# SZU-AdvTech-2022/165-Learning-based-Multi-modality-Image-and-Video-Compression

Hardware: AMD Instinct MI355X
Metric: 256×256 patches/sec (RD-loss fwd+bwd) at 1/2/4/8 GPUs; PSNR/bpp parity (higher is better)
Workload: dtype bf16; 1 GPU; bmshj2018-hyperprior q1 B=16 256x256 RD-loss training step (fwd+bwd+clip+Adam+aux), HIP-graph replay; model=bmshj2018-hyperprior, quality=1, global_batch=16, per_gpu_batch=16, patch=256, parallelism=dp1

## Files before the change

### 165-learning-based-multi-modality-image-and-video-compression_amd/compressai/_native.py

```python
from __future__ import annotations

import ctypes
import os
from ctypes import POINTER, Structure, c_char_p, c_float, c_int, c_int32, c_int64, c_size_t, c_void_p

_PKG_ROOT = os.path.dirname(os.path.dirname(os.path.abspath(__file__)))
LIB_PATH = os.environ.get("CAI_LIB", os.path.join(_PKG_ROOT, "lib", "libcai.so"))

CAI_OK, CAI_EINVAL, CAI_EDEVICE, CAI_EWORKSPACE = 0, 1, 2, 3
F32, BF16 = 0, 1
ACT_NONE, ACT_RELU, ACT_LEAKY = 0, 1, 2
MASK_NONE, MASK_POS, MASK_LEAKY, MASK_SIGN = 0, 1, 2, 3
MASK_BEFORE_RES = 16
Q_NOISE, Q_DEQUANTIZE, Q_SYMBOLS = 0, 1, 2
ADAM_CLIP, ADAM_SKIP_NONFINITE, ADAM_ZERO_GRAD = 1, 2, 4
ADAM_SMALL_N = 1 << 16


class ConvGeom(Structure):
    _fields_ = [(n, c_int32) for n in (
        "batch", "in_c", "in_h", "in_w", "out_c", "out_h", "out_w",
        "kernel", "stride", "pad", "output_padding", "transposed")]


# ... 62 lines not shown
                ("out", c_void_p), ("gc", c_void_p), ("gb", c_void_p), ("ga", c_void_p), ("res2", c_void_p),
                ("xmask", c_void_p), ("x_ld", c_int32), ("y_ld", c_int32), ("out_ld", c_int32),
                ("res2_ld", c_int32), ("xmask_ld", c_int32), ("kpa", c_int32), ("kpb", c_int32), ("kpc", c_int32),
                ("gy_masked", c_int32)]


class ResunitWgradArgs(Structure):
    _fields_ = [("batch", c_int32), ("h", c_int32), ("w", c_int32), ("n", c_int32),
                ("x", c_void_p), ("h1", c_void_p), ("h2", c_void_p), ("ga", c_void_p), ("gb", c_void_p),
                ("gc", c_void_p), ("x_ld", c_int32), ("gc_ld", c_int32), ("dwa", c_void_p), ("dba", c_void_p),
                ("dwb", c_void_p), ("dbb", c_void_p), ("dwc", c_void_p), ("dbc", c_void_p), ("accumulate", c_int32)]


_P, _I, _I64, _F, _S = c_void_p, c_int, c_int64, c_float, c_size_t
_G = POINTER(ConvGeom)
_N = POINTER(NoiseSrc)
SIGNATURES = {
    "cai_last_error": (c_char_p, []),
    "cai_version": (c_int, []),
    "cai_abi_count": (c_int, []),
    "cai_conv_packed_weight_bytes": (_S, [_G, _I, _I]),
    "cai_conv_pack_weight": (_I, [_G, _I, _I, _P, _P, _P, _P]),
    "cai_conv_pack_desc_bytes": (_S, []),
    "cai_conv_pack_describe": (_I, [_G, _I, _I, _P, _P, _P, _P]),
    "cai_conv_pack_finalize": (_I64, [_P, c_int32]),
    "cai_conv_pack_many": (_I, [_P, c_int32, _I, _I64, _P]),
    "cai_pack_nchw": (_I, [_P, c_int32, c_int32, c_int32, c_int32, _I, _P, c_int32, _P]),
    "cai_conv_workspace_bytes": (_S, [_G, _I, _I]),
    "cai_conv_fwd": (_I, [_G, _I, _P, c_int32, c_int32, _P, _P, c_int32, _F, _P, _I, _I64, _I64, _I64, _I64,
                          _P, _S, _P]),
    "cai_conv_fwd_res": (_I, [_G, _I, _P, c_int32, c_int32, _P, _P, c_int32, _F, _P, c_int32, _P, _I, _I64, _I64,
                              _I64, _I64, _P, _S, _P]),
    "cai_conv_gdn_fwd": (_I, [_G, _I, _P, c_int32, c_int32, _P, _P, _P, _I64, _I64, _I64, _I64, _P, _P, c_int32, _P,
                              c_int32, _P, _S, _P]),
    "cai_conv_gdn_fused": (c_int32, [_G, _I, c_int32]),
    "cai_conv_gdn_kernel_name": (c_char_p, [_G, _I, c_int32, c_int32]),
    "cai_conv_dgrad": (_I, [_G, _I, _P, c_int32, _P, _P, c_int32, c_int32, _F, _P, c_int32, _P, _S, _P]),
    "cai_conv_dgrad_res": (_I, [_G, _I, _P, c_int32, _P, _P, c_int32, _P, c_int32, c_int32, _F, _P, c_int32, _P, _S,
                                _P]),
    "cai_conv_dgrad_res2": (_I, [_G, _I, _P, c_int32, _P, _P, c_int32, _P, c_int32, _P, c_int32, c_int32, _F, _P,
                                 c_int32, _P, _S, _P]),
    "cai_conv_wgrad_workspace_bytes": (_S, [_G, _I]),
    "cai_resunit": (_I, [POINTER(ResunitArgs), c_int32, _P]),
    "cai_resunit_wgrad_workspace_bytes": (_S, [POINTER(ResunitWgradArgs)]),
    "cai_resunit_wgrad": (_I, [POINTER(ResunitWgradArgs), _P, _S, _P, POINTER(ReduceJob)]),
    "cai_conv_kernel_name": (c_char_p, [_G, _I, _I, c_int32]),
    "cai_conv_split_factor": (c_int32, [_G, _I, _I, c_int32]),
    "cai_conv_wgrad": (_I, [_G, _I, _P, c_int32, c_int32, c_int32, _P, c_int32, _P, _P, c_int32, _P, _S, _P]),
    "cai_conv_wgrad_deferred": (_I, [_G, _I, _P, c_int32, c_int32, c_int32, _P, c_int32, _P, _P, c_int32, _P, _S, _P,
                                     POINTER(ReduceJob)]),
    "cai_reduce_jobs": (_I, [POINTER(ReduceJob), c_int32, _P]),
    "cai_reduce_jobs_grid": (_I, [POINTER(ReduceJob), c_int32, c_int32, _P]),
    "cai_conv_wgrad_batch": (_I, [POINTER(WgradCall), c_int32, _P, POINTER(ReduceJob)]),
    "cai_resunit_wgrad_batch": (_I, [POINTER(ResunitWgradArgs), POINTER(c_void_p), POINTER(c_size_t), c_int32, _P,
                                    POINTER(ReduceJob)]),
    "cai_deconv_small_workspace_bytes": (_S, [_G, _I]),
    "cai_deconv_small_fwd": (_I, [_G, _I, _P, c_int32, _P, _P, _P, _P, _S, _P]),
    "cai_deconv_small_bwd": (_I, [_G, _I, _P, c_int32, _P, _P, _P, c_int32, _P, _P, c_int32, _P, _S, _P]),
    "cai_edge_supported": (_I, [_G, _I]),
    "cai_edge_workspace_bytes": (_S, [_G, _I]),
    "cai_edge_frag_bytes": (_S, [_G, _I, _I]),
    "cai_edge_pack_weights": (_I, [_G, _I, _I, _P, _P, _P]),
    "cai_edge_pack_describe": (_I, [_G, _I, _I, _P, _P, _P]),
    "cai_edge_conv_fwd": (_I, [_G, _P, _P, _P, _P, c_int32, _P]),
    "cai_edge_conv_gdn_fwd": (_I, [_G, _P, _P, _P, _P, c_int32, _P, _P, _P, c_int32, _P]),
    "cai_edge_conv_gdn_fused": (c_int32, [_G]),
    "cai_edge_deconv_fwd": (_I, [_G, _P, c_int32, _P, _P, _P, _P]),
    "cai_edge_deconv_dgrad": (_I, [_G, _P, _P, _P, c_int32, _P]),
    "cai_edge_wgrad": (_I, [_G, _P, _P, c_int32, _P, _P, c_int32, _P, _S, _P]),
    "cai_edge_wgrad_deferred": (_I, [_G, _P, _P, c_int32, _P, _P, c_int32, _P, _S, _P, POINTER(ReduceJob)]),
    "cai_add_act": (_I, [_I, _P, c_int32, _P, c_int32, _P, c_int32, _I64, c_int32, c_int32, _F, _P]),
    "cai_axpy_dev": (_I, [_I64, _P, _P, _P, _P]),
    "cai_act": (_I, [_I, _P, c_int32, _P, c_int32, _I64, c_int32, c_int32, _F, _P]),
    "cai_gdn1_out": (_I, [_I, _P, c_int32, _P, c_int32, _P, c_int32, _I64, c_int32, c_int32, _P]),
    "cai_gdn1_out_bwd": (_I, [_I, _P, c_int32, _P, c_int32, _P, c_int32, _P, c_int32, _P, c_int32, _I64, c_int32,
                              c_int32, _P]),
    "cai_gate_fwd": (_I, [_I, _P, _P, _P, _P, c_int32, _I64, c_int32, _P]),
    "cai_gate_bwd": (_I, [_I, _P, _P, _P, c_int32, _P, _P, c_int32, _I64, c_int32, c_int32, _P]),
    "cai_pixel_shuffle": (_I, [_I, _P, POINTER(c_int64), _P, POINTER(c_int64), c_int32, c_int32, c_int32, c_int32,
                               c_int32, c_int32, _P]),
    "cai_layernorm_fwd": (_I, [_I, _P, c_int32, _I64, c_int32, _P, _P, _F, _P, c_int32, _P, _P, _P]),
    "cai_layernorm_bwd_workspace_bytes": (_S, [_I64, c_int32]),
    "cai_layernorm_bwd": (_I, [_I, _P, c_int32, _P, c_int32, _I64, c_int32, _P, _P, _P, _P, c_int32, _P, _P, c_int32,
                               _P, _S, _P]),
    "cai_gelu_fwd": (_I, [_I, _P, c_int32, _P, c_int32, _I64, c_int32, _P]),
    "cai_gelu_bwd": (_I, [_I, _P, c_int32, _P, c_int32, _P, c_int32, _I64, c_int32, _P]),
    "cai_window_attn_fwd": (_I, [_I, POINTER(WindowAttn), _P, c_int32, _P]),
    "cai_window_attn_bwd_workspace_bytes": (_S, [POINTER(WindowAttn)]),
    "cai_window_attn_bwd": (_I, [_I, POINTER(WindowAttn), _P, c_int32, _P, c_int32, _P, c_int32, _P, c_int32, _P, _S,
                                 _P]),
    "cai_channel_mean_workspace_bytes": (_S, [c_int32, _I64, c_int32]),
    "cai_channel_mean": (_I, [_I, _P, c_int32, _P, c_int32, c_int32, _I64, c_int32, _P, _F, _P, _S, _P]),
    "cai_channel_affine": (_I, [_I, _P, c_int32, _P, _P, _F, _P, c_int32, c_int32, _I64, c_int32, _P]),
    "cai_gdn_reparam": (_I, [_P, _P, c_int32, _F, _F, _I, _P, _P, _P]),
    "cai_gdn_reparam_describe": (_I, [_P, _P, c_int32, _F, _F, _P, _P, _P]),
    "cai_gdn_fwd": (_I, [_I, _P, c_int32, _I64, c_int32, _P, _P, c_int32, _P, c_int32, _P]),
    "cai_gdn_bwd": (_I, [_I, _P, c_int32, _P, c_int32, _I64, c_int32, _P, _P, c_int32, _P, c_int32, _P, _P]),
    "cai_gdn_param_grad_workspace_bytes": (_S, [_I64, c_int32, _I]),
    "cai_gdn_param_grad": (_I, [_I, _P, c_int32, _P, _I64, c_int32, _P, _P, _F, _F, _P, _P, c_int32, _P, _S, _P]),
    "cai_gdn_backward_workspace_bytes": (_S, [_I64, c_int32, _I]),
    "cai_gdn_kernel_name": (c_char_p, [_I, _I64, c_int32, c_int32, c_int32, c_int32]),
    "cai_gdn_backward": (_I, [_I, _P, c_int32, _P, c_int32, _I64, c_int32, _P, _P, c_int32, _P, c_int32, _P, _P, _F, _F,
                              _P, _P, c_int32, _P, _S, _P]),
    "cai_gdn_backward_deferred": (_I, [_I, _P, c_int32, _P, c_int32, _I64, c_int32, _P, _P, c_int32, _P, c_int32, _P,
                                       _P, _F, _F, _P, _P, c_int32, _P, _S, _P, POINTER(ReduceJob)]),
    "cai_uniform_noise": (_I, [_P, _I64, _P, _P]),
# ... 83 lines not shown
```

### 165-learning-based-multi-modality-image-and-video-compression_amd/compressai/_ops.py

```python
from __future__ import annotations

import ctypes
import math
import os
import warnings
from typing import Optional, Sequence, Tuple

import torch

from . import _ledger
from ._native import (ACT_LEAKY, ACT_NONE, ACT_RELU, BF16, F32, MASK_BEFORE_RES, MASK_LEAKY, MASK_NONE, MASK_POS,
                      Q_DEQUANTIZE, Q_NOISE,
                      GC_SCALES_RELU, JOB_EDGE, JOB_GDN, JOB_NONE, JOB_WGRAD, NOISE_BUF, NOISE_DRAW, NOISE_REPLAY, ArArgs, ConvGeom, EbGrads, EbParams, NoiseSrc, RdGrads,
                      RdInputs, ReduceJob, ResunitArgs, ResunitWgradArgs, WgradCall, lib)

_VP = ctypes.c_void_p
_GDN_TWO_PASS = os.environ.get("CAI_GDN_TWO_PASS", "0") == "1"
_RD_UNFUSED = os.environ.get("CAI_RD_UNFUSED", "0") == "1"
_EDGE_OFF = os.environ.get("CAI_EDGE_OFF", "0") == "1"



DIRECT_GRAD_ATTR = "_cai_direct_grad"

# ... 703 lines not shown
            fan, done = getattr(ctx, "fan", None), False
            if fan is not None and fan.pending is not None and dres is None and dt == torch.bfloat16 and ldx % 8 == 0:
                post = fan.pending
                if aux is None:
                    dres, fan.pending = post, None
                elif "halo" not in _conv_kernel(g, dt, 1)():
                    ppm, pld = to_pm(post, dt, 4)
                    mode = spec.in_mask | MASK_BEFORE_RES
                    _ledger.run(lambda ppm=ppm, dx=dx, wt=wt, gpm=gpm, ws=ws: lib.cai_conv_dgrad_res(
                                    ctypes.byref(g), code, _p(gpm), gld, _p(wt), _p(ppm), pld, _p(dx), ldx, mode,
                                    spec.in_mask_param, _p(xpm), ctx.xld, _p(ws), wsb, st),
                                "conv_dgrad", _conv_kernel(g, dt, 1), fl, nb + post.numel() * _es(dt), dt,
                                _ledger.shape_of(g))
                    fan.pending, done = None, True
            if done:
                pass
            elif dres is not None and dt == torch.bfloat16 and aux is None and ldx % 8 == 0:
                rpm, rld = to_pm(dres, dt, 4)
                maux = xpm if rmask != MASK_NONE else None
                if dres2 is not None:
                    r2pm, r2ld = to_pm(dres2, dt, 4)
                    _ledger.run(lambda: lib.cai_conv_dgrad_res2(ctypes.byref(g), code, _p(gpm), gld, _p(wt), _p(rpm),
                                                                rld, _p(r2pm), r2ld, _p(dx), ldx, rmask, 0.0,
                                                                _p(maux), ctx.xld if maux is not None else 0, _p(ws),
                                                                wsb, st),
                                "conv_dgrad", _conv_kernel(g, dt, 1), fl, nb, dt, _ledger.shape_of(g))
                else:
                    _ledger.run(lambda: lib.cai_conv_dgrad_res(ctypes.byref(g), code, _p(gpm), gld, _p(wt), _p(rpm),
                                                               rld, _p(dx), ldx, rmask, 0.0, _p(maux),
                                                               ctx.xld if maux is not None else 0, _p(ws), wsb, st),
                                "conv_dgrad", _conv_kernel(g, dt, 1), fl, nb, dt, _ledger.shape_of(g))
            else:
                _ledger.run(lambda: lib.cai_conv_dgrad(ctypes.byref(g), code, _p(gpm), gld, _p(wt), _p(dx), ldx,
                                                       spec.in_mask, spec.in_mask_param, _p(aux),
                                                       ctx.xld if aux is not None else 0, _p(ws), wsb, st),
                            "conv_dgrad", _conv_kernel(g, dt, 1), fl, nb, dt, _ledger.shape_of(g))
                if dres is not None:
                    dx = dx + dres
                if dres2 is not None:
                    dx = dx + dres2
                if rmask != MASK_NONE:
                    raise RuntimeError("conv dgrad: a residual-gradient mask needs the fused bf16 path")
        if ctx.needs_input_grad[1] or (ctx.has_bias and ctx.needs_input_grad[2]):
            wparam, bparam = ctx.params
            dw, db = conv_wgrad(g, dt, xpm, ctx.xld, int(spec.in_abs), gpm, gld, wparam, bparam, weight,
                                ctx.has_bias)
        dres = None
        if ctx.has_res and ctx.needs_input_grad[4]:
            dres = gpm
        return dx, dw, db, None, dres


_BATCHED_WGRAD = {}
_BATCHED_WGRAD_KERNELS = (b"wgrad_small_kernel", b"wgrad_glds_kernel<256>", b"wgrad_glds_kernel<128>",
                          b"wgrad_halo_kernel<3,s1>")


def _small_wgrad(g, code, in_abs) -> bool:
    key = (tuple(getattr(g, f) for f, _ in ConvGeom._fields_), code, int(in_abs))
    v = _BATCHED_WGRAD.get(key)
    if v is None:
        name = lib.cai_conv_kernel_name(ctypes.byref(g), code, 2, int(in_abs))
        v = _BATCHED_WGRAD[key] = name in _BATCHED_WGRAD_KERNELS
    return v


def conv_wgrad(g, dt, xpm, xld, in_abs, gpm, gld, wparam, bparam, weight, has_bias):
    code = dcode(dt)
    dev = gpm.device
    nbytes = lib.cai_conv_wgrad_workspace_bytes(ctypes.byref(g), code)
    wbase = getattr(wparam, "_base", None)
    wdir = wparam if direct_grad(wparam) else (
        wbase if wbase is not None and wbase.numel() == wparam.numel() and direct_grad(wbase) else None)
    direct = wdir is not None and (bparam is None or direct_grad(bparam))
    if direct:
        dw = wdir.grad if wdir is wparam else wdir.grad.view(wparam.shape)
        db = bparam.grad if bparam is not None else None
    else:
        dw = torch.empty(weight.shape, dtype=torch.float32, device=dev)
        db = torch.empty(g.out_c, dtype=torch.float32, device=dev) if has_bias else None
    fl, nb = _ledger.conv_cost(g, _es(dt), 2)
    st = _stream()
    if defer_reduce_ok(direct) and _WGRAD_BATCH and not _WGRAD_SIDE_PX and _small_wgrad(g, code, in_abs):
        wws = torch.empty(nbytes, dtype=torch.uint8, device=dev)
        call = WgradCall(g, code, _p(xpm), xld, int(in_abs), 0, _p(gpm), gld, _p(dw), _p(db), 1, _p(wws), nbytes)
        defer_wgrad_call(call, dev, xpm, gpm, wws)
    elif defer_reduce_ok(direct):
        npix = g.batch * (g.in_h * g.in_w if g.transposed else g.out_h * g.out_w)
        with _SideDeferred(dev, npix, xpm, gpm):
            wws = torch.empty(nbytes, dtype=torch.uint8, device=dev)
            job = ReduceJob()
            lib.cai_conv_wgrad_deferred(ctypes.byref(g), code, _p(xpm), xld, int(in_abs), 0, _p(gpm), gld, _p(dw),
                                        _p(db), 1, _p(wws), nbytes, _stream(), ctypes.byref(job))
            defer_job(job, dev, wws)
    else:
        with _WgradLaunch(dev, direct, xpm, gpm):
            wws = torch.empty(nbytes, dtype=torch.uint8, device=dev)
            sw = _stream()
            _ledger.run(lambda: lib.cai_conv_wgrad(ctypes.byref(g), code, _p(xpm), xld, int(in_abs), 0, _p(gpm), gld,
                                                   _p(dw), _p(db), int(direct), _p(wws), nbytes, sw),
                        "conv_wgrad", _conv_kernel(g, dt, 2, in_abs), fl, nb, dt, _ledger.shape_of(g))
    if direct:
        return None, None
    if weight.dtype != torch.float32:
        dw = dw.to(weight.dtype)
    return dw, db


# ... 1491 lines not shown
```

### 165-learning-based-multi-modality-image-and-video-compression_amd/csrc/conv.hip

```cpp
#include "common.hpp"

#include <type_traits>
#include "edge_frag.hpp"
#include "gdn_tile.hpp"
#include "mfma.hpp"
#include "reduce_jobs.hpp"
#include "conv_args.hpp"

#include <algorithm>
#include <vector>

namespace cai {

constexpr int NT = 256;


__device__ __forceinline__ int swz(int row, int slot) { return slot ^ ((row >> 1) & 7); }

__device__ __forceinline__ float apply_act(float v, int act, float prm) {
    if (act == CAI_ACT_RELU) return v > 0.f ? v : 0.f;
    if (act == CAI_ACT_LEAKY) return v > 0.f ? v : v * prm;
    return v;
}
__device__ __forceinline__ float act_pre(const ConvArgs& a, float v) {
// ... 3116 lines not shown
        one(std::integral_constant<int, 1>());
        one(std::integral_constant<int, 2>());
        one(std::integral_constant<int, 3>());
    }
    if constexpr ((FLAGS & WG_BIAS) != 0) {
        if (do_bias) {
#pragma unroll
            for (int tm = 0; tm < TMR; ++tm) {
                if ((tm & 3) != wc) continue;
                float v = bsum[tm];
                v += __shfl_xor(v, 16);
                v += __shfl_xor(v, 32);
                const int n = r0 + wr * (16 * TMR) + tm * 16 + lane;
                if (lane < 16 && n < a.Ng) a.bws[(int64_t)split * a.Ng + n] = v;
            }
        }
    }
    if constexpr ((FLAGS & WG_TBIAS) != 0) {
#pragma unroll
        for (int t = 0; t < W::TN; ++t) {
            float v = tsum[t];
            v += __shfl_xor(v, 16);
            v += __shfl_xor(v, 32);
            const int col = wcol + t * 16 + (lane & 15);
            if (lane < 16 && tsel[t] >= 0)
                a.bws[((int64_t)split * a.tb_s * a.tb_s + tsel[t]) * a.nbias + q0 + col % 64] = v;
        }
    }
#pragma unroll
    for (int tn = 0; tn < W::TN; ++tn) {
        const int col = wcol + tn * 16 + (lane & 15), kw = col / 64;
        const int gcol = (kh * KS + kw) * a.Cq_pad + q0 + col % 64;
#pragma unroll
        for (int tm = 0; tm < TMR; ++tm)
#pragma unroll
            for (int r = 0; r < 4; ++r) {
                const int row = r0 + wr * (16 * TMR) + tm * 16 + (lane >> 4) * 4 + r;
                if (row < a.Ng) out[(int64_t)row * a.ncols + gcol] = acc[tm][tn][r];
            }
    }
}

template <int KS, int S, int FLAGS, int R = 1, int TMR = 4>
__global__ __launch_bounds__(512, 1) void wgrad_halo_kernel(const WgradArgs a) {
    __shared__ __attribute__((aligned(16))) char smem[WhCfg<KS, S, R, TMR == 6 ? 192 : 128>::BYTES];
    wgrad_halo_block<KS, S, FLAGS, R, TMR>(a, (int)blockIdx.x, (int)gridDim.x, smem);
}

template <int KS, int S, int FLAGS, int R = 1, int TMR = 4>
__global__ __launch_bounds__(512, 1) void wgrad_halo_batch_kernel(const WgBatch b) {
    __shared__ __attribute__((aligned(16))) char smem[WhCfg<KS, S, R, TMR == 6 ? 192 : 128>::BYTES];
    const int L = (int)blockIdx.x, j = wg_batch_job(b, L), l = L - b.start[j];
    if (l < b.nwg[j]) wgrad_halo_block<KS, S, FLAGS, R, TMR>(b.job[j], l, b.nwg[j], smem);
}

template <int KS, int S, int R = 1, int TMR = 4>
static void launch_wgrad_halo(const WgradArgs& a, int nblocks, int bias, hipStream_t st) {
    if (bias == WG_BIAS)
        hipLaunchKernelGGL((wgrad_halo_kernel<KS, S, WG_BIAS, R, TMR>), dim3(nblocks), dim3(512), 0, st, a);
    else if (S == 2 && bias == WG_TBIAS)
        hipLaunchKernelGGL((wgrad_halo_kernel<KS, S, WG_TBIAS, R, TMR>), dim3(nblocks), dim3(512), 0, st, a);
    else
        hipLaunchKernelGGL((wgrad_halo_kernel<KS, S, 0, R, TMR>), dim3(nblocks), dim3(512), 0, st, a);
}

template <int KS, int S, int R = 1, int TMR = 4>
static void launch_wgrad_halo_batch(const WgBatch& b, int bias, hipStream_t st) {
    const dim3 grid(b.start[b.n]);
    if (bias == WG_BIAS)
        hipLaunchKernelGGL((wgrad_halo_batch_kernel<KS, S, WG_BIAS, R, TMR>), grid, dim3(512), 0, st, b);
    else if (S == 2 && bias == WG_TBIAS)
        hipLaunchKernelGGL((wgrad_halo_batch_kernel<KS, S, WG_TBIAS, R, TMR>), grid, dim3(512), 0, st, b);
    else
        hipLaunchKernelGGL((wgrad_halo_batch_kernel<KS, S, 0, R, TMR>), grid, dim3(512), 0, st, b);
}

template <int CT>
static void launch_wgrad_glds_batch(const WgBatch& b, int f, hipStream_t st) {
    const dim3 grid(b.start[b.n]);
    switch (f) {
        case WG_TBIAS: hipLaunchKernelGGL((wgrad_glds_batch_kernel<CT, WG_TBIAS>), grid, dim3(512), 0, st, b); break;
        case 0: hipLaunchKernelGGL((wgrad_glds_batch_kernel<CT, 0>), grid, dim3(512), 0, st, b); break;
        case WG_ABS: hipLaunchKernelGGL((wgrad_glds_batch_kernel<CT, WG_ABS>), grid, dim3(512), 0, st, b); break;
        case WG_SQ: hipLaunchKernelGGL((wgrad_glds_batch_kernel<CT, WG_SQ>), grid, dim3(512), 0, st, b); break;
        case WG_BIAS: hipLaunchKernelGGL((wgrad_glds_batch_kernel<CT, WG_BIAS>), grid, dim3(512), 0, st, b); break;
        case WG_ABS | WG_BIAS:
            hipLaunchKernelGGL((wgrad_glds_batch_kernel<CT, WG_ABS | WG_BIAS>), grid, dim3(512), 0, st, b);
            break;
        default:
            hipLaunchKernelGGL((wgrad_glds_batch_kernel<CT, WG_SQ | WG_BIAS>), grid, dim3(512), 0, st, b);
            break;
    }
}

template <int CT>
static void launch_wgrad_glds(const WgradArgs& a, int nblocks, int in_abs, int in_sq, int bias, hipStream_t st) {
    const int f = (in_abs ? WG_ABS : 0) | (in_sq ? WG_SQ : 0) | bias;
    switch (f) {
        case WG_TBIAS: hipLaunchKernelGGL((wgrad_glds_kernel<CT, WG_TBIAS>), dim3(nblocks), dim3(512), 0, st, a); break;
        case 0: hipLaunchKernelGGL((wgrad_glds_kernel<CT, 0>), dim3(nblocks), dim3(512), 0, st, a); break;
        case WG_ABS: hipLaunchKernelGGL((wgrad_glds_kernel<CT, WG_ABS>), dim3(nblocks), dim3(512), 0, st, a); break;
        case WG_SQ: hipLaunchKernelGGL((wgrad_glds_kernel<CT, WG_SQ>), dim3(nblocks), dim3(512), 0, st, a); break;
        case WG_BIAS: hipLaunchKernelGGL((wgrad_glds_kernel<CT, WG_BIAS>), dim3(nblocks), dim3(512), 0, st, a); break;
        case WG_ABS | WG_BIAS:
            hipLaunchKernelGGL((wgrad_glds_kernel<CT, WG_ABS | WG_BIAS>), dim3(nblocks), dim3(512), 0, st, a);
            break;
// ... 1396 lines not shown
            return CAI_OK;
        }
        return launch_reduce_jobs(&J, 1, st);
    }
    float* bws = nullptr;
    if (W.glds) {
        int key, nblocks;
        wgrad_split_setup(g, W, a, workspace, db, in_abs, in_sq, key, nblocks);
        bws = a.bws;
        launch_wgrad_split(a, key, nblocks, st);
    } else {
        dim3 grid(8 * a.ctiles * a.rtiles * a.nsub);
        if (dtype == CAI_BF16)
            hipLaunchKernelGGL(wgrad_kernel<bf16>, grid, dim3(NT), 0, st, a);
        else
            hipLaunchKernelGGL(wgrad_kernel<float>, grid, dim3(NT), 0, st, a);
    }
    a.bws = bws;
    const cai_reduce_job J = wgrad_split_job(g, W, a, dw, db, accumulate);
    (void)slab;
    if (job) {
        *job = J;
    } else {
        rc = launch_reduce_jobs(&J, 1, st);
        if (rc) return rc;
    }
    if (db && !bws) {
        float* part = reinterpret_cast<float*>(reinterpret_cast<char*>(workspace) + W.ws_slab + W.ws_bias);
        const int64_t npix = (int64_t)g->batch * g->out_h * g->out_w;
        if (dtype == CAI_BF16)
            launch_colsum<bf16>(dy, npix, g->out_c, dy_ld, W.nchunk, W.chunk, part, db, accumulate, st);
        else
            launch_colsum<float>(dy, npix, g->out_c, dy_ld, W.nchunk, W.chunk, part, db, accumulate, st);
    }
    CAI_LAUNCH_CHECK("conv_wgrad");
    return CAI_OK;
}

int cai_conv_wgrad(const cai_conv_geom* g, int dtype, const void* x, int32_t x_ld, int32_t in_abs, int32_t in_sq,
                   const void* dy, int32_t dy_ld, float* dw, float* db, int32_t accumulate, void* workspace,
                   size_t ws_bytes, void* stream) {
    return run_conv_wgrad(g, dtype, x, x_ld, in_abs, in_sq, dy, dy_ld, dw, db, accumulate, workspace, ws_bytes, stream,
                          nullptr);
}

int cai_conv_wgrad_deferred(const cai_conv_geom* g, int dtype, const void* x, int32_t x_ld, int32_t in_abs,
                            int32_t in_sq, const void* dy, int32_t dy_ld, float* dw, float* db, int32_t accumulate,
                            void* workspace, size_t ws_bytes, void* stream, cai_reduce_job* job) {
    CAI_CHECK_ARG(job, "conv_wgrad_deferred: null job");
    return run_conv_wgrad(g, dtype, x, x_ld, in_abs, in_sq, dy, dy_ld, dw, db, accumulate, workspace, ws_bytes, stream,
                          job);
}

int cai_conv_wgrad_batch(const cai_wgrad_call* calls, int32_t n, void* stream, cai_reduce_job* jobs) {
    CAI_CHECK_ARG(n >= 0 && (n == 0 || (calls && jobs)), "conv_wgrad_batch: bad arguments");
    hipStream_t st = as_stream(stream);
    SwBatch b[6];
    for (int c = 0; c < 6; ++c) b[c].n = 0, b[c].start[0] = 0;
    std::vector<std::pair<int, WgBatch>> groups;
    for (int i = 0; i < n; ++i) {
        const cai_wgrad_call& c = calls[i];
        jobs[i] = cai_reduce_job{};
        if (!small_wgrad_ok(&c.geom, c.dtype)) {
            WgradPlan W;
            WgradArgs a;
            int rc = wgrad_prepare(&c.geom, c.dtype, c.x, c.x_ld, c.in_abs, c.in_sq, c.dy, c.dy_ld, c.dw, c.db,
                                   c.workspace, c.ws_bytes, W, a);
            if (rc) return rc;
            const bool fused_bias = !c.db || ((W.fused_bias || W.tbias));
            if (!W.glds || !fused_bias) {
                rc = run_conv_wgrad(&c.geom, c.dtype, c.x, c.x_ld, c.in_abs, c.in_sq, c.dy, c.dy_ld, c.dw, c.db,
                                    c.accumulate, c.workspace, c.ws_bytes, stream, &jobs[i]);
                if (rc) return rc;
                continue;
            }
            int key, nblocks;
            wgrad_split_setup(&c.geom, W, a, c.workspace, c.db, c.in_abs, c.in_sq, key, nblocks);
            jobs[i] = wgrad_split_job(&c.geom, W, a, c.dw, c.db, c.accumulate);
            size_t gi = 0;
            while (gi < groups.size() && groups[gi].first != key) ++gi;
            if (gi == groups.size()) {
                groups.emplace_back(key, WgBatch{});
                groups[gi].second.n = 0;
                groups[gi].second.start[0] = 0;
            }
            WgBatch& B = groups[gi].second;
            if (B.n == WG_BATCH_MAX) {
                launch_wgrad_split_batch(B, key, st);
                B.n = 0;
            }
            B.job[B.n] = a;
            B.nwg[B.n] = nblocks;
            B.start[B.n + 1] = B.start[B.n] + (nblocks + 7) / 8 * 8;
            ++B.n;
            continue;
        }
        WgradPlan W;
        WgradArgs a;
        int rc = wgrad_prepare(&c.geom, c.dtype, c.x, c.x_ld, c.in_abs, c.in_sq, c.dy, c.dy_ld, c.dw, c.db,
                               c.workspace, c.ws_bytes, W, a);
        if (rc) return rc;
        SwArgs sa;
        dim3 grid;
        rc = small_wgrad_setup(&c.geom, W, a, c.dy, c.dy_ld, c.dw, c.db, c.accumulate, a.ws, sa, grid, jobs[i]);
        if (rc) return rc;
        const bool lng = W.M > SW_NW * SW_STEPS * 32;
        const int cls = (sa.in_abs ? 1 : (sa.in_sq ? 2 : 0)) + (lng ? 3 : 0);
        SwBatch& B = b[cls];
        bool clash = false;
        for (int j = 0; j < B.n; ++j) clash |= sa.db && B.job[j].db == sa.db;
        if (clash || B.n == SW_BATCH_MAX) {
            launch_wgrad_small_batch(B, cls, st);
            B.n = 0;
        }
        B.job[B.n] = sa;
        B.gx[B.n] = (int)grid.x;
        B.gy[B.n] = (int)grid.y;
        B.start[B.n + 1] = B.start[B.n] + (int)(grid.x * grid.y);
        ++B.n;
    }
    for (int c = 0; c < 6; ++c)
        if (b[c].n) launch_wgrad_small_batch(b[c], c, st);
    for (auto& kv : groups)
        if (kv.second.n) launch_wgrad_split_batch(kv.second, kv.first, st);
    CAI_LAUNCH_CHECK("conv_wgrad_batch");
    return CAI_OK;
}

}

namespace cai {
int colsum_any(int dtype, const void* g, int64_t npix, int C, int ld, float* out, int accumulate, void* ws,
               size_t wsb, hipStream_t st) {
    const int nchunk = colsum_nchunk(npix);
    const int64_t chunk = (npix + nchunk - 1) / nchunk;
    CAI_CHECK_ARG(wsb >= (size_t)nchunk * C * sizeof(float), "colsum: workspace too small");
    CAI_CHECK_ARG(C <= COLSUM_MAXC && ld % (dtype == CAI_BF16 ? 8 : 4) == 0, "colsum: bad layout");
    if (dtype == CAI_BF16)
        launch_colsum<bf16>(g, npix, C, ld, nchunk, chunk, reinterpret_cast<float*>(ws), out, accumulate, st);
    else
        launch_colsum<float>(g, npix, C, ld, nchunk, chunk, reinterpret_cast<float*>(ws), out, accumulate, st);
    return CAI_OK;
}
size_t colsum_ws_bytes(int64_t npix, int C) { return (size_t)colsum_nchunk(npix) * C * sizeof(float); }
}
```

### 165-learning-based-multi-modality-image-and-video-compression_amd/csrc/optim.hip

```cpp
#include "common.hpp"

#include <stdarg.h>

namespace cai {

static thread_local char g_err[512] = "";

void set_error(const char* fmt, ...) {
    va_list ap;
    va_start(ap, fmt);
    vsnprintf(g_err, sizeof(g_err), fmt, ap);
    va_end(ap);
}

__global__ void adam_kernel(float* __restrict__ p, const float* __restrict__ g, float* __restrict__ m,
                            float* __restrict__ v, int64_t n, float lr, float b1, float b2, float eps,
                            const float* __restrict__ step, const float* __restrict__ sqnorm, float max_norm) {
    if (sqnorm && !isfinite(*sqnorm)) return;
    const float t = *step + 1.f;
    const float bc1 = 1.f - powf(b1, t);
    const float bc2s = sqrtf(1.f - powf(b2, t));
    const float step_size = lr / bc1;
    float scale = 1.f;
    if (sqnorm) {
// ... 119 lines not shown
                                                         float* __restrict__ sqnorm_out, float max_norm, int zero_g) {
    __shared__ float red[4];
    float acc = 0.f;
    for (int i = threadIdx.x; i < nparts; i += 256) acc += part[i];
    const float sq = block_sum_all<256>(acc, red);
    const bool lead = blockIdx.x == 0 && threadIdx.x == 0;
    if (lead && sqnorm_out) *sqnorm_out = sq;
    const int64_t i0 = blockIdx.x * (int64_t)blockDim.x + threadIdx.x, stride = (int64_t)gridDim.x * blockDim.x;
    if (!isfinite(sq)) {
        if (lead) *step -= 1.f;
        if (zero_g) zero_range(g, n, i0, stride);
        return;
    }
    const float t = *step;
    const float coef = max_norm / (sqrtf(sq) + 1e-6f);
    adam_range(p, g, m, v, n, i0, stride, coef < 1.f ? coef : 1.f, b1, b2, eps, lr / (1.f - powf(b1, t)),
               sqrtf(1.f - powf(b2, t)), zero_g != 0);
}

__global__ __launch_bounds__(1024) void adam_small_kernel(float* __restrict__ p, float* __restrict__ g,
                                                          float* __restrict__ m, float* __restrict__ v, int64_t n,
                                                          float lr, float b1, float b2, float eps, float* step,
                                                          float* __restrict__ sqnorm_out, float max_norm,
                                                          int use_norm, int zero_g) {
    __shared__ float red[16];
    float scale = 1.f;
    if (use_norm) {
        float acc = 0.f;
        for (int64_t i = threadIdx.x; i < n; i += 1024) acc += g[i] * g[i];
        const float sq = block_sum_all<1024>(acc, red);
        if (threadIdx.x == 0 && sqnorm_out) *sqnorm_out = sq;
        if (!isfinite(sq)) {
            if (zero_g) zero_range(g, n, threadIdx.x, 1024);
            return;
        }
        const float coef = max_norm / (sqrtf(sq) + 1e-6f);
        scale = coef < 1.f ? coef : 1.f;
    }
    const float t = *step + 1.f;
    __syncthreads();
    adam_range(p, g, m, v, n, threadIdx.x, 1024, scale, b1, b2, eps, lr / (1.f - powf(b1, t)),
               sqrtf(1.f - powf(b2, t)), zero_g != 0);
    if (threadIdx.x == 0) *step = t;
}

}

using namespace cai;

extern "C" {

const char* cai_last_error(void) { return g_err; }
int cai_version(void) { return 1; }
int cai_abi_count(void) { return 103; }

int cai_adam(float* p, const float* g, float* m, float* v, int64_t n, float lr, float beta1, float beta2, float eps,
             float* step, const float* sqnorm, float max_norm, void* stream) {
    CAI_CHECK_ARG(p && g && m && v && step, "adam: null pointer");
    CAI_CHECK_ARG(((uintptr_t)p | (uintptr_t)g | (uintptr_t)m | (uintptr_t)v) % 16 == 0, "adam: buffers must be 16-byte aligned");
    if (n > 0) {
        int64_t blocks = (n / 4 + 255) / 256;
        if (blocks > 2048) blocks = 2048;
        if (blocks < 1) blocks = 1;
        hipLaunchKernelGGL(adam_kernel, dim3((unsigned)blocks), dim3(256), 0, as_stream(stream), p, g, m, v, n, lr,
                           beta1, beta2, eps, step, sqnorm, max_norm);
    }
    hipLaunchKernelGGL(step_incr_kernel, dim3(1), dim3(1), 0, as_stream(stream), step, sqnorm);
    CAI_LAUNCH_CHECK("adam");
    return CAI_OK;
}

size_t cai_adam_step_workspace_bytes(int64_t n) { return (size_t)sq_parts(n) * sizeof(float); }

int cai_adam_step(float* p, float* g, float* m, float* v, int64_t n, float lr, float beta1, float beta2,
                  float eps, float* step, float* sqnorm, float max_norm, int32_t flags, void* workspace,
                  size_t ws_bytes, void* stream) {
    CAI_CHECK_ARG(p && g && m && v && step && n >= 0, "adam_step: bad arguments");
    CAI_CHECK_ARG(((uintptr_t)p | (uintptr_t)g | (uintptr_t)m | (uintptr_t)v) % 16 == 0,
                  "adam_step: buffers must be 16-byte aligned");
    const bool clip = (flags & CAI_ADAM_CLIP) != 0, use_norm = clip || (flags & CAI_ADAM_SKIP_NONFINITE);
    const int zero_g = (flags & CAI_ADAM_ZERO_GRAD) ? 1 : 0;
    const float mn = clip ? max_norm : INFINITY;
    hipStream_t st = as_stream(stream);
    if (n <= ADAM_SMALL_N) {
        hipLaunchKernelGGL(adam_small_kernel, dim3(1), dim3(1024), 0, st, p, g, m, v, n, lr, beta1, beta2, eps, step,
                           sqnorm, mn, (int)use_norm, zero_g);
    } else if (!use_norm) {
        CAI_CHECK_ARG(!zero_g, "adam_step: ZERO_GRAD needs CLIP or SKIP_NONFINITE above the one-block size");
        return cai_adam(p, g, m, v, n, lr, beta1, beta2, eps, step, nullptr, INFINITY, stream);
    } else {
        CAI_CHECK_ARG(workspace && ws_bytes >= cai_adam_step_workspace_bytes(n), "adam_step: workspace too small");
        const int np = sq_parts(n);
        float* part = reinterpret_cast<float*>(workspace);
        hipLaunchKernelGGL(sq_part_kernel, dim3(np), dim3(256), 0, st, g, n, part, step);
        int64_t blocks = (n / 4 + 255) / 256;
        blocks = blocks > 2048 ? 2048 : (blocks < 1 ? 1 : blocks);
        hipLaunchKernelGGL(adam_fused_kernel, dim3((unsigned)blocks), dim3(256), 0, st, p, g, m, v, n, lr, beta1,
                           beta2, eps, step, part, np, sqnorm, mn, zero_g);
    }
    CAI_LAUNCH_CHECK("adam_step");
    return CAI_OK;
}

}
```

### include/cai.h

```cpp
#ifndef CAI_H
#define CAI_H

#include <stddef.h>
#include <stdint.h>

#ifdef __cplusplus
extern "C" {
#endif

#define CAI_OK 0
#define CAI_EINVAL 1
#define CAI_EDEVICE 2
#define CAI_EWORKSPACE 3

#define CAI_F32 0
#define CAI_BF16 1

#define CAI_ACT_NONE 0
#define CAI_ACT_RELU 1
#define CAI_ACT_LEAKY 2

#define CAI_MASK_NONE 0
#define CAI_MASK_POS 1
#define CAI_MASK_LEAKY 2
// ... 92 lines not shown
    void* out;
    void* gc;
    void* gb;
    void* ga;
    const void* res2;
    const void* xmask;
    int32_t x_ld, y_ld, out_ld, res2_ld, xmask_ld;
    int32_t kpa, kpb, kpc;
    int32_t gy_masked;
} cai_resunit_args;
int cai_resunit(const cai_resunit_args* args, int32_t direction, void* stream);

const char* cai_conv_kernel_name(const cai_conv_geom* g, int dtype, int direction, int32_t in_abs);
int32_t cai_conv_split_factor(const cai_conv_geom* g, int dtype, int direction, int32_t in_abs);

size_t cai_conv_wgrad_workspace_bytes(const cai_conv_geom* g, int dtype);
int cai_conv_wgrad(const cai_conv_geom* g, int dtype,
                   const void* x, int32_t x_ld, int32_t in_abs, int32_t in_sq,
                   const void* dy, int32_t dy_ld,
                   float* dw, float* db, int32_t accumulate,
                   void* workspace, size_t ws_bytes, void* stream);

#define CAI_JOB_NONE 0
#define CAI_JOB_WGRAD 1
#define CAI_JOB_GDN 2
#define CAI_JOB_EDGE 3
typedef struct cai_reduce_job {
    int32_t kind, nblocks;
    int32_t i[10];
    float f[2];
    const void* p[6];
} cai_reduce_job;
int cai_conv_wgrad_deferred(const cai_conv_geom* g, int dtype,
                            const void* x, int32_t x_ld, int32_t in_abs, int32_t in_sq,
                            const void* dy, int32_t dy_ld,
                            float* dw, float* db, int32_t accumulate,
                            void* workspace, size_t ws_bytes, void* stream, cai_reduce_job* job);
int cai_reduce_jobs(const cai_reduce_job* jobs, int32_t n, void* stream);
int cai_reduce_jobs_grid(const cai_reduce_job* jobs, int32_t n, int32_t max_blocks, void* stream);
typedef struct cai_wgrad_call {
    cai_conv_geom geom;
    int32_t dtype;
    const void* x;
    int32_t x_ld, in_abs, in_sq;
    const void* dy;
    int32_t dy_ld;
    float* dw;
    float* db;
    int32_t accumulate;
    void* workspace;
    size_t ws_bytes;
} cai_wgrad_call;
int cai_conv_wgrad_batch(const cai_wgrad_call* calls, int32_t n, void* stream, cai_reduce_job* jobs);

typedef struct cai_resunit_wgrad_args {
    int32_t batch, h, w, n;
    const void* x;
    const void* h1;
    const void* h2;
    const void* ga;
    const void* gb;
    const void* gc;
    int32_t x_ld, gc_ld;
    float* dwa;
    float* dba;
    float* dwb;
    float* dbb;
    float* dwc;
    float* dbc;
    int32_t accumulate;
} cai_resunit_wgrad_args;
size_t cai_resunit_wgrad_workspace_bytes(const cai_resunit_wgrad_args* args);
int cai_resunit_wgrad_batch(const cai_resunit_wgrad_args* args, void* const* workspaces, const size_t* ws_bytes,
                            int32_t n, void* stream, cai_reduce_job* jobs);
int cai_resunit_wgrad(const cai_resunit_wgrad_args* args, void* workspace, size_t ws_bytes, void* stream,
                      cai_reduce_job* jobs);

size_t cai_deconv_small_workspace_bytes(const cai_conv_geom* g, int dtype);
int cai_deconv_small_fwd(const cai_conv_geom* g, int dtype, const void* x, int32_t x_ld,
                         const float* w, const float* bias, float* y,
                         void* workspace, size_t ws_bytes, void* stream);
int cai_deconv_small_bwd(const cai_conv_geom* g, int dtype, const void* x, int32_t x_ld,
                         const float* w, const float* dy, void* dx, int32_t dx_ld,
                         float* dw, float* db, int32_t accumulate,
                         void* workspace, size_t ws_bytes, void* stream);

int cai_edge_supported(const cai_conv_geom* g, int dtype);
size_t cai_edge_workspace_bytes(const cai_conv_geom* g, int dtype);
size_t cai_edge_frag_bytes(const cai_conv_geom* g, int dtype, int direction);
int cai_edge_pack_weights(const cai_conv_geom* g, int dtype, int direction, const float* w, void* frag,
                          void* stream);
int cai_edge_pack_describe(const cai_conv_geom* g, int dtype, int direction, const float* w, void* frag,
                           void* desc);
int cai_edge_conv_fwd(const cai_conv_geom* g, const float* x, const void* frag, const float* bias, void* y,
                      int32_t y_ld, void* stream);
int cai_edge_conv_gdn_fwd(const cai_conv_geom* g, const float* x, const void* frag, const float* bias, void* xo,
                          int32_t xo_ld, const void* gamma_op, const float* beta, void* y, int32_t y_ld,
                          void* stream);
int32_t cai_edge_conv_gdn_fused(const cai_conv_geom* g);
int cai_edge_deconv_fwd(const cai_conv_geom* g, const void* x, int32_t x_ld, const void* frag, const float* bias,
                        float* y, void* stream);
int cai_edge_deconv_dgrad(const cai_conv_geom* g, const float* dy, const void* frag, void* dx, int32_t dx_ld,
                          void* stream);
int cai_edge_wgrad(const cai_conv_geom* g, const float* img, const void* feat, int32_t feat_ld, float* dw, float* db,
                   int32_t accumulate, void* workspace, size_t ws_bytes, void* stream);
int cai_edge_wgrad_deferred(const cai_conv_geom* g, const float* img, const void* feat, int32_t feat_ld, float* dw,
// ... 244 lines not shown
```

Measured before the change: 10680 patches/s.

## Batch heterogeneous 5x5 stride-2 halo wgrad jobs into one mixed-variant launch

Adds a wgrad_halo_mix_kernel that dispatches per job to different 5x5 stride-2 halo wgrad template variants (rows per block, tile height, bias mode). This lets those jobs be routed into the batched wgrad path and share a single launch. A host-side planner can also rebalance split counts across jobs using a cost model, so the jobs finish together within the block budget. The aim is fewer kernel launches and better GPU fill for small wgrad convolutions. The cost is a kernel with a runtime switch, shared memory sized for the largest variant, and changed split factors that alter workspace use.

Measured after the change: 10690 patches/s (median of 3 runs). About the same (+0.1%).

```diff
diff --git a/165-learning-based-multi-modality-image-and-video-compression_amd/compressai/_native.py b/165-learning-based-multi-modality-image-and-video-compression_amd/compressai/_native.py
--- a/165-learning-based-multi-modality-image-and-video-compression_amd/compressai/_native.py
+++ b/165-learning-based-multi-modality-image-and-video-compression_amd/compressai/_native.py
@@ -138,6 +138,7 @@
     "cai_reduce_jobs": (_I, [POINTER(ReduceJob), c_int32, _P]),
     "cai_reduce_jobs_grid": (_I, [POINTER(ReduceJob), c_int32, c_int32, _P]),
     "cai_conv_wgrad_batch": (_I, [POINTER(WgradCall), c_int32, _P, POINTER(ReduceJob)]),
+    "cai_conv_wgrad_mix_plan": (_I, [POINTER(WgradCall), c_int32, POINTER(c_int32), POINTER(c_int32)]),
     "cai_resunit_wgrad_batch": (_I, [POINTER(ResunitWgradArgs), POINTER(c_void_p), POINTER(c_size_t), c_int32, _P,
                                     POINTER(ReduceJob)]),
     "cai_deconv_small_workspace_bytes": (_S, [_G, _I]),
diff --git a/165-learning-based-multi-modality-image-and-video-compression_amd/compressai/_ops.py b/165-learning-based-multi-modality-image-and-video-compression_amd/compressai/_ops.py
--- a/165-learning-based-multi-modality-image-and-video-compression_amd/compressai/_ops.py
+++ b/165-learning-based-multi-modality-image-and-video-compression_amd/compressai/_ops.py
@@ -779,8 +779,11 @@
 
 
 _BATCHED_WGRAD = {}
+_WGRAD_MIX = os.environ.get("CAI_WGRAD_MIX", "1") != "0"
 _BATCHED_WGRAD_KERNELS = (b"wgrad_small_kernel", b"wgrad_glds_kernel<256>", b"wgrad_glds_kernel<128>",
                           b"wgrad_halo_kernel<3,s1>")
+if _WGRAD_MIX:
+    _BATCHED_WGRAD_KERNELS += (b"wgrad_halo_kernel<5,r2>", b"wgrad_halo_kernel<5,r4>")
 
 
 def _small_wgrad(g, code, in_abs) -> bool:
diff --git a/165-learning-based-multi-modality-image-and-video-compression_amd/csrc/conv.hip b/165-learning-based-multi-modality-image-and-video-compression_amd/csrc/conv.hip
--- a/165-learning-based-multi-modality-image-and-video-compression_amd/csrc/conv.hip
+++ b/165-learning-based-multi-modality-image-and-video-compression_amd/csrc/conv.hip
@@ -3192,6 +3192,37 @@
     __shared__ __attribute__((aligned(16))) char smem[WhCfg<KS, S, R, TMR == 6 ? 192 : 128>::BYTES];
     const int L = (int)blockIdx.x, j = wg_batch_job(b, L), l = L - b.start[j];
     if (l < b.nwg[j]) wgrad_halo_block<KS, S, FLAGS, R, TMR>(b.job[j], l, b.nwg[j], smem);
+}
+
+struct WgMix {
+    WgBatch b;
+    int var[WG_BATCH_MAX];
+};
+static_assert(sizeof(WgMix) <= 4096, "kernel argument block");
+
+constexpr int wg_mix_smem() {
+    return WhCfg<5, 2, 2>::BYTES > WhCfg<5, 2, 4>::BYTES ? WhCfg<5, 2, 2>::BYTES : WhCfg<5, 2, 4>::BYTES;
+}
+
+__global__ __launch_bounds__(512, 1) void wgrad_halo_mix_kernel(const WgMix m) {
+    __shared__ __attribute__((aligned(16))) char smem[wg_mix_smem()];
+    const int L = (int)blockIdx.x, j = wg_batch_job(m.b, L), l = L - m.b.start[j], n = m.b.nwg[j];
+    if (l >= n) return;
+    const WgradArgs& a = m.b.job[j];
+    switch (m.var[j]) {
+        case 0: wgrad_halo_block<5, 2, 0, 2, 4>(a, l, n, smem); break;
+        case 1: wgrad_halo_block<5, 2, WG_BIAS, 2, 4>(a, l, n, smem); break;
+        case 2: wgrad_halo_block<5, 2, WG_TBIAS, 2, 4>(a, l, n, smem); break;
+        case 3: wgrad_halo_block<5, 2, 0, 2, 2>(a, l, n, smem); break;
+        case 4: wgrad_halo_block<5, 2, WG_BIAS, 2, 2>(a, l, n, smem); break;
+        case 5: wgrad_halo_block<5, 2, WG_TBIAS, 2, 2>(a, l, n, smem); break;
+        case 6: wgrad_halo_block<5, 2, 0, 4, 4>(a, l, n, smem); break;
+        case 7: wgrad_halo_block<5, 2, WG_BIAS, 4, 4>(a, l, n, smem); break;
+        case 8: wgrad_halo_block<5, 2, WG_TBIAS, 4, 4>(a, l, n, smem); break;
+        case 9: wgrad_halo_block<5, 2, 0, 4, 2>(a, l, n, smem); break;
+        case 10: wgrad_halo_block<5, 2, WG_BIAS, 4, 2>(a, l, n, smem); break;
+        default: wgrad_halo_block<5, 2, WG_TBIAS, 4, 2>(a, l, n, smem); break;
+    }
 }
 
 template <int KS, int S, int R = 1, int TMR = 4>
@@ -4694,9 +4725,148 @@
                           job);
 }
 
+static int wgrad_mix_mode() {
+    const char* e = getenv("CAI_WGRAD_MIX");
+    return (e && *e == '0') ? 0 : ((e && *e == '2') ? 2 : 1);
+}
+constexpr double WG_MIX_STRIP_US[2] = {1.2, 1.11};
+constexpr double WG_MIX_FIXED_US[2] = {13.0, 8.4};
+
+static bool wgrad_mix_shareable(const cai_wgrad_call& c, const WgradPlan& W) {
+    const int R = halo_wgrad_rows(&c.geom);
+    return W.halo == 5 && c.geom.stride == 2 && (R == 2 || R == 4) && (W.hrows == 128 || W.hrows == 64) &&
+           (!c.db || W.fused_bias || W.tbias);
+}
+
+struct WgMixSlot {
+    int launch = -1;
+    int S = 0, strips_per_split = 0, tiles = 0;
+    double us = 0.0;
+};
+
+static void plan_wgrad_mix(const cai_wgrad_call* calls, int n, std::vector<WgMixSlot>& slot) {
+    slot.assign((size_t)n, WgMixSlot{});
+    const int mode = wgrad_mix_mode();
+    if (!mode) return;
+    std::vector<int> idx;
+    std::vector<WgradPlan> plan;
+    for (int i = 0; i < n; ++i) {
+        const cai_wgrad_call& c = calls[i];
+        if (check_geom(&c.geom) || (c.dtype != CAI_BF16 && c.dtype != CAI_F32) || small_wgrad_ok(&c.geom, c.dtype))
+            continue;
+        const WgradPlan W = make_wgrad_plan(&c.geom, c.dtype, true, c.in_abs || c.in_sq);
+        if (!wgrad_mix_shareable(c, W)) continue;
+        idx.push_back(i);
+        plan.push_back(W);
+    }
+    const int budget = wg_blocks();
+    for (size_t b0 = 0, launch = 0; b0 < idx.size(); b0 += WG_BATCH_MAX) {
+        const size_t b1 = std::min(idx.size(), b0 + WG_BATCH_MAX);
+        if (b1 - b0 < 2) break;
+        auto nstrip = [&](size_t j) { return plan[j].M / 64; };
+        auto us = [&](size_t j, int64_t strips) {
+            const int h = plan[j].hrows == 64;
+            return WG_MIX_FIXED_US[h] + (double)strips * WG_MIX_STRIP_US[h];
+        };
+        if (mode == 1) {
+            for (size_t j = b0; j < b1; ++j) {
+                WgMixSlot& s = slot[(size_t)idx[j]];
+                s.launch = (int)launch;
+                s.tiles = plan[j].tiles;
+                s.S = plan[j].S;
+                s.strips_per_split = plan[j].strips_per_split;
+                s.us = us(j, s.strips_per_split);
+            }
+            ++launch;
+            continue;
+        }
+        auto smax = [&](size_t j) { return (int)std::max<int64_t>(1, nstrip(j) / wg_min_strips()); };
+        auto splits_at = [&](size_t j, double T, int& S, int& sps) {
+            const int h = plan[j].hrows == 64;
+            const int64_t m = std::min<int64_t>(nstrip(j), (int64_t)((T - WG_MIX_FIXED_US[h]) / WG_MIX_STRIP_US[h] + 1e-6));
+            if (m < 1 || (nstrip(j) + m - 1) / m > smax(j)) return false;
+            S = (int)((nstrip(j) + m - 1) / m);
+            sps = (int)((nstrip(j) + S - 1) / S);
+            S = (int)((nstrip(j) + sps - 1) / sps);
+            return true;
+        };
+        auto blocks_at = [&](double T) {
+            int sum = 0, S, sps;
+            for (size_t j = b0; j < b1; ++j) {
+                if (!splits_at(j, T, S, sps)) return -1;
+                sum += S * plan[j].tiles;
+            }
+            return sum;
+        };
+        double best = 0.0, solo = 0.0;
+        for (size_t j = b0; j < b1; ++j) {
+            best = std::max(best, us(j, nstrip(j)));
+            solo += us(j, plan[j].strips_per_split);
+        }
+        for (size_t j = b0; j < b1; ++j)
+            for (int S = 1; S <= smax(j) && S * plan[j].tiles <= budget; ++S) {
+                const double T = us(j, (nstrip(j) + S - 1) / S);
+                if (T >= best) continue;
+                const int sum = blocks_at(T);
+                if (sum >= 0 && sum <= budget) best = T;
+            }
+        const int sum = blocks_at(best);
+        if (sum < 0 || sum > budget || best >= solo) continue;
+        for (size_t j = b0; j < b1; ++j) {
+            WgMixSlot& s = slot[(size_t)idx[j]];
+            s.launch = (int)launch;
+            s.tiles = plan[j].tiles;
+            splits_at(j, best, s.S, s.strips_per_split);
+            s.us = us(j, s.strips_per_split);
+        }
+        ++launch;
+    }
+}
+
+static std::vector<int> wgrad_mix_order(const std::vector<WgMixSlot>& slot) {
+    std::vector<int> ord;
+    for (size_t i = 0; i < slot.size(); ++i)
+        if (slot[i].launch >= 0) ord.push_back((int)i);
+    std::stable_sort(ord.begin(), ord.end(), [&](int a, int b) {
+        const WgMixSlot &x = slot[(size_t)a], &y = slot[(size_t)b];
+        return x.launch != y.launch ? x.launch < y.launch : x.us > y.us;
+    });
+    return ord;
+}
+
+static int wgrad_mix_var(const cai_conv_geom* g, const WgradPlan& W, int bflag) {
+    return (halo_wgrad_rows(g) == 4 ? 6 : 0) + (W.hrows == 64 ? 3 : 0) + (bflag == WG_BIAS ? 1 : bflag == WG_TBIAS ? 2 : 0);
+}
+
+int cai_conv_wgrad_mix_plan(const cai_wgrad_call* calls, int32_t n, int32_t* plan, int32_t* limits) {
+    CAI_CHECK_ARG(n >= 0 && (n == 0 || (calls && plan)), "conv_wgrad_mix_plan: bad arguments");
+    std::vector<WgMixSlot> slot;
+    plan_wgrad_mix(calls, n, slot);
+    for (int i = 0; i < n; ++i) {
+        const WgMixSlot& s = slot[(size_t)i];
+        int32_t* o = plan + 5 * i;
+        o[0] = s.launch; o[1] = s.S; o[2] = s.strips_per_split; o[3] = 0; o[4] = s.S * s.tiles;
+    }
+    int launch = -1, next = 0;
+    for (int i : wgrad_mix_order(slot)) {
+        if (slot[(size_t)i].launch != launch) launch = slot[(size_t)i].launch, next = 0;
+        plan[5 * i + 3] = next;
+        next += (plan[5 * i + 4] + 7) / 8 * 8;
+    }
+    if (limits) limits[0] = wg_blocks(), limits[1] = wg_min_strips();
+    return CAI_OK;
+}
+
 int cai_conv_wgrad_batch(const cai_wgrad_call* calls, int32_t n, void* stream, cai_reduce_job* jobs) {
     CAI_CHECK_ARG(n >= 0 && (n == 0 || (calls && jobs)), "conv_wgrad_batch: bad arguments");
     hipStream_t st = as_stream(stream);
+    std::vector<WgMixSlot> slot;
+    plan_wgrad_mix(calls, n, slot);
+    struct MixJob {
+        WgradArgs a;
+        int nblocks, var;
+    };
+    std::vector<MixJob> mixjob((size_t)n);
     SwBatch b[6];
     for (int c = 0; c < 6; ++c) b[c].n = 0, b[c].start[0] = 0;
     std::vector<std::pair<int, WgBatch>> groups;
@@ -4717,6 +4887,21 @@
                 continue;
             }
             int key, nblocks;
+            const WgMixSlot& ms = slot[(size_t)i];
+            if (ms.launch >= 0) {
+                CAI_CHECK_ARG(ms.S >= 1 && ms.S <= W.S, "conv_wgrad_batch: shared plan with more splits than solo");
+                W.S = ms.S;
+                W.strips_per_split = ms.strips_per_split;
+                W.ws_slab = (size_t)W.S * W.Ng * W.ncols * sizeof(float);
+                W.Sb = W.fused_bias ? W.S : (W.tbias ? W.S * c.geom.stride * c.geom.stride : 0);
+                W.ws_bias = W.Sb ? ((size_t)W.Sb * W.nbias * sizeof(float) + 255) / 256 * 256 : 0;
+                CAI_CHECK_ARG(c.ws_bytes >= W.ws_slab + W.ws_bias + W.ws_col + 256,
+                              "conv_wgrad_batch: workspace too small for the shared plan");
+                wgrad_split_setup(&c.geom, W, a, c.workspace, c.db, c.in_abs, c.in_sq, key, nblocks);
+                jobs[i] = wgrad_split_job(&c.geom, W, a, c.dw, c.db, c.accumulate);
+                mixjob[(size_t)i] = MixJob{a, nblocks, wgrad_mix_var(&c.geom, W, key & (WG_BIAS | WG_TBIAS))};
+                continue;
+            }
             wgrad_split_setup(&c.geom, W, a, c.workspace, c.db, c.in_abs, c.in_sq, key, nblocks);
             jobs[i] = wgrad_split_job(&c.geom, W, a, c.dw, c.db, c.accumulate);
             size_t gi = 0;
@@ -4765,6 +4950,22 @@
         if (b[c].n) launch_wgrad_small_batch(b[c], c, st);
     for (auto& kv : groups)
         if (kv.second.n) launch_wgrad_split_batch(kv.second, kv.first, st);
+    WgMix M{};
+    int launch = -1;
+    auto flush_mix = [&] {
+        if (M.b.n) hipLaunchKernelGGL(wgrad_halo_mix_kernel, dim3(M.b.start[M.b.n]), dim3(512), 0, st, M);
+        M.b.n = 0;
+    };
+    for (int i : wgrad_mix_order(slot)) {
+        if (slot[(size_t)i].launch != launch) flush_mix(), launch = slot[(size_t)i].launch;
+        const MixJob& j = mixjob[(size_t)i];
+        M.b.job[M.b.n] = j.a;
+        M.b.nwg[M.b.n] = j.nblocks;
+        M.b.start[M.b.n + 1] = M.b.start[M.b.n] + (j.nblocks + 7) / 8 * 8;
+        M.var[M.b.n] = j.var;
+        ++M.b.n;
+    }
+    flush_mix();
     CAI_LAUNCH_CHECK("conv_wgrad_batch");
     return CAI_OK;
 }
diff --git a/165-learning-based-multi-modality-image-and-video-compression_amd/csrc/optim.hip b/165-learning-based-multi-modality-image-and-video-compression_amd/csrc/optim.hip
--- a/165-learning-based-multi-modality-image-and-video-compression_amd/csrc/optim.hip
+++ b/165-learning-based-multi-modality-image-and-video-compression_amd/csrc/optim.hip
@@ -195,7 +195,7 @@
 
 const char* cai_last_error(void) { return g_err; }
 int cai_version(void) { return 1; }
-int cai_abi_count(void) { return 103; }
+int cai_abi_count(void) { return 104; }
 
 int cai_adam(float* p, const float* g, float* m, float* v, int64_t n, float lr, float beta1, float beta2, float eps,
              float* step, const float* sqnorm, float max_norm, void* stream) {
diff --git a/include/cai.h b/include/cai.h
--- a/include/cai.h
+++ b/include/cai.h
@@ -168,6 +168,7 @@
     size_t ws_bytes;
 } cai_wgrad_call;
 int cai_conv_wgrad_batch(const cai_wgrad_call* calls, int32_t n, void* stream, cai_reduce_job* jobs);
+int cai_conv_wgrad_mix_plan(const cai_wgrad_call* calls, int32_t n, int32_t* plan, int32_t* limits);
 
 typedef struct cai_resunit_wgrad_args {
     int32_t batch, h, w, n;
```
